# JvanZyl1/PSSO-SAC-for-powered-descent

Measured on AMD Instinct MI355X. Metric: env-steps/sec at 65 536 parallel envs; achieved HBM GB/s vs peak, higher is better.
Workload: dtype f64; 1 GPU; c3: 65536 envs/GPU, landing_burn_pure_throttle, rtd_rl reward, wind (percentile profile drawn per reset + VK gusts below 15 km) + tilt, auto-reset, uniform random actions; synchronized starts, 640 untimed burn-in + 5 warmup steps; envs_per_gpu=65536, global_envs=65536, parallelism=env-shard x1

## Files before the change

### include/pdenv.h

```cpp
#ifndef PDENV_H
#define PDENV_H
#include <stddef.h>
#include <stdint.h>

#ifdef __cplusplus
extern "C" {
#endif

#define PD_ABI_VERSION 11
#define PD_MAX_PTS 256
#define PD_MAX_COLS 5
#define PD_MAX_TAB 64
#define PD_MAX_WIND 16
#define PD_N_WIND_PROFILES 50
#define PD_N_STATE 11
#define PD_N_INFO 49
#define PD_ACTOR_PARAMS_PURE_THROTTLE 249
#define PD_ACTOR_PARAMS_LANDING_BURN 372

typedef enum { PD_OK = 0, PD_ERR_INVALID = 1, PD_ERR_HIP = 2, PD_ERR_NOMEM = 3, PD_ERR_UNSUPPORTED = 4 } pd_status;
typedef enum {
    PD_PHASE_PURE_THROTTLE = 0, PD_PHASE_LANDING_BURN = 1, PD_PHASE_PCONTROL = 2,
    PD_PHASE_BALLISTIC_ARC = 3, PD_PHASE_FLIP_OVER = 4, PD_PHASE_SUBSONIC = 5, PD_PHASE_SUPERSONIC = 6,
    PD_PHASE_LANDING_BURN_ACS = 7
} pd_phase;
typedef enum { PD_RTD_RL = 0, PD_RTD_PSO = 1, PD_RTD_NONE = 2 } pd_rtd;
typedef enum { PD_F64 = 0, PD_F32 = 1 } pd_precision;
typedef enum { PD_INTEG_REFERENCE = 0, PD_INTEG_RK4 = 1 } pd_integrator;
typedef enum {
    PD_TABLES_NO_CELL_PIECES = 1,
    PD_TABLES_NO_FINE_INDEX = 2,
    PD_TABLES_EXACT_ATMOSPHERE = 4,
    PD_TABLES_VERBOSE = 8,
    PD_TABLES_NO_CARRY = 16,
    PD_TABLES_NO_ATM_LDS = 32
} pd_table_flags;

typedef struct {
    int32_t n_cols, n_pts;
    double col_aoa[PD_MAX_COLS];
    int32_t col_start[PD_MAX_COLS], col_len[PD_MAX_COLS];
    double mach[PD_MAX_PTS];
    double coef[PD_MAX_PTS];
} pd_aero_table;

typedef struct {
    double thrust_per_engine, nozzle_exit_pressure, nozzle_exit_area, v_exhaust;
    int32_t n_engines_gimballed, pad0;
    double grid_fin_area, d_base_grid_fin, rocket_radius, frontal_area, m_prop0, C_gust_x, C_gust_y;
    double h_ox, h_f, m_ox, m_f, h_lower, m_dry, x_dry, I_dry, engine_height, cop;
    double isa_Hb[9], isa_Tb[9], isa_beta[9], isa_pb[9];
    double isa_g0, isa_R, isa_kappa, isa_r, isa_alt_max, grav_R, grav_g0;
    pd_aero_table cd, cl;
    int32_t ca_n, cn_n;
    double ca_x[PD_MAX_TAB], ca_y[PD_MAX_TAB], ca_min_mach, ca_min_val;
    double cn_x[PD_MAX_TAB], cn_y[PD_MAX_TAB], cn_min_mach, cn_max_mach, cn_min_val, cn_max_val, cn_slope;
    int32_t wind_n[PD_N_WIND_PROFILES];
    double wind_alt_km[PD_N_WIND_PROFILES][PD_MAX_WIND], wind_speed[PD_N_WIND_PROFILES][PD_MAX_WIND];
    double vk_Ad_u[4], vk_Bd_u[2], vk_Ad_v[4], vk_Bd_v[2], vk_y_threshold;
    double sigma_u_lo, sigma_u_hi, sigma_v_lo, sigma_v_hi;
    double state0[PD_N_STATE];
    double norm_y, norm_vy, norm_x, norm_vx;
    const uint64_t* keys_cd; int64_t n_keys_cd;
    const uint64_t* keys_cl; int64_t n_keys_cl;
    double full_rocket[13];
    double cop_ascent;
    int32_t n_engines_stage1, pad1;
    double rcs_force, rcs_d_bottom, rcs_d_top;
// ... 183 lines not shown
```

### psso-sac-for-powered-descent_amd/csrc/kstep.hip

```cpp
#include "pd_step_impl.h"

#if !defined(PD_KR) || !defined(PD_KPH) || !defined(PD_KW)
#error "kstep.hip needs -DPD_KR=0|1 -DPD_KPH=0|1|2 -DPD_KW=0|1"
#endif

namespace pd {
#if PD_KR == 0
using KR = double;
#else
using KR = float;
#endif
constexpr bool KW = PD_KW != 0;

#define PD_INST_STEP(RT)                                                          \
    template void launch_step<KR, PD_KPH, RT, KW, 1>(const StepArgs<KR>&, hipStream_t);  \
    template void launch_step<KR, PD_KPH, RT, KW, 2>(const StepArgs<KR>&, hipStream_t);  \
    template void launch_step<KR, PD_KPH, RT, KW, 4>(const StepArgs<KR>&, hipStream_t);  \
    template void launch_step<KR, PD_KPH, RT, KW, 8>(const StepArgs<KR>&, hipStream_t);  \
    template void launch_step<KR, PD_KPH, RT, KW, 16>(const StepArgs<KR>&, hipStream_t);

#if defined(PD_KROLL)
static_assert(PD_KPH < 2, "SAC rollout unit: the two landing burns");
#if PD_KROLL == 2
template void launch_sac_collect<KR, PD_KPH, KW>(const StepArgs<KR>&, hipStream_t);
#else
template void launch_sac_roll<KR, PD_KPH, KW>(const StepArgs<KR>&, hipStream_t);
#endif
#elif defined(PD_KRK4)
static_assert(PD_KPH == 0 && PD_KW == 0, "RK4 unit: pure throttle without wind");
template void launch_step<KR, 0, 0, false, 2, true>(const StepArgs<KR>&, hipStream_t);
template void launch_step<KR, 0, 0, false, 16, true>(const StepArgs<KR>&, hipStream_t);
template void launch_step<KR, 0, 1, false, 2, true>(const StepArgs<KR>&, hipStream_t);
template void launch_step<KR, 0, 1, false, 16, true>(const StepArgs<KR>&, hipStream_t);
#elif defined(PD_KLPE)
template void launch_step<KR, PD_KPH, 0, KW, PD_KLPE>(const StepArgs<KR>&, hipStream_t);
#else
PD_INST_STEP(0)
#endif
#if PD_KPH < 2 && !defined(PD_KLPE) && !defined(PD_KRK4) && !defined(PD_KROLL)
PD_INST_STEP(1)
template void launch_policy_lpe<KR, PD_KPH, KW, 2>(const StepArgs<KR>&, int64_t, hipStream_t);
template void launch_policy_lpe<KR, PD_KPH, KW, 4>(const StepArgs<KR>&, int64_t, hipStream_t);
template void launch_policy_lpe<KR, PD_KPH, KW, 8>(const StepArgs<KR>&, int64_t, hipStream_t);
#endif
}
```

### psso-sac-for-powered-descent_amd/csrc/pd_step.h

```cpp
#pragma once
#include <hip/hip_runtime.h>

#include <cstring>

#include "../../include/pdenv.h"
#include "pd_physics.h"
#include "pd_sac_mlp.h"

namespace pd {

constexpr int kBlock = 256;
constexpr int kStepBlock = 256;
#ifndef PD_WG512
#define PD_WG512 1
#endif
#ifndef PD_ATM_LDS
#define PD_ATM_LDS 1
#endif
#ifndef PD_WIND_SLOPE
#define PD_WIND_SLOPE 1
#endif
#ifndef PD_MERGE
#define PD_MERGE 2
#endif
template <typename R, int PHASE, bool WIND, int LPE, int POL, bool RK4, bool SAC> constexpr bool step_big() {
    return PD_WG512 != 0 && sizeof(R) == 8 && PHASE == 0 && WIND && LPE == 2 && POL == 0 && !RK4 && !SAC;
}
template <typename R, int PHASE, bool WIND, int LPE, int POL, bool RK4, bool SAC> constexpr int step_block() {
    return step_big<R, PHASE, WIND, LPE, POL, RK4, SAC>() ? 512 : kStepBlock;
}
constexpr int kScratch = kSys * kSys + kSys + 3 * kNbr + kPay;
constexpr int kPendingCap = 4096;
constexpr int kSolveSlots = 1024;
constexpr int kGridExact = 1 << 30;
constexpr int kGridRefine = 1 << 29;
constexpr int kGridBisect = 1 << 28;
constexpr int kGridPiece = 1 << 27;
constexpr uint32_t kFinePiece = 1u << 30;
constexpr uint32_t kFineBisect = 1u << 29;
constexpr uint32_t kFineRefined = 1u << 28;
constexpr uint32_t kFineIndex = kFineRefined - 1u;

constexpr int kCellDeg = 8;
constexpr int kCellCoef = (kCellDeg + 1) * (kCellDeg + 2) / 2;
constexpr int kCellExact = 4;
constexpr int kCellKey = kCellCoef + 3 * kCellExact;
constexpr int kCellStride = (kCellKey + 2) & ~1;
constexpr int kCellKeyF = (kCellKey + 1) & ~1;
constexpr int kCellStrideF = (kCellKeyF + 2 + 3) & ~3;
template <typename R> constexpr int cell_stride() { return sizeof(R) == 8 ? kCellStride : kCellStrideF; }
template <typename R> constexpr int cell_key() { return sizeof(R) == 8 ? kCellKey : kCellKeyF; }

struct GridBisect {
    double nx, ny, c, tau;
    unsigned long long key_a, key_b;
    int slot_a, slot_b;
// ... 136 lines not shown
    unsigned int* ticket;
};

template <typename R>
__device__ void insert_pending(unsigned long long* count, const unsigned long long* pkeys, const double* ppay,
                               unsigned long long* stats, unsigned long long* keys_cd, R* pay_cd, int lc_cd,
                               unsigned long long* keys_cl, R* pay_cl, int lc_cl) {
    unsigned long long cnt = *count;
    if (cnt == 0) return;
    if (cnt > (unsigned long long)kPendingCap) cnt = kPendingCap;
    for (unsigned long long e = 0; e < cnt; ++e) {
        const unsigned long long kk = pkeys[e];
        const int table = (int)(kk >> 63);
        const unsigned long long key = kk & ~(1ull << 63);
        unsigned long long* keys = table ? keys_cl : keys_cd;
        const int lc = table ? lc_cl : lc_cd;
        uint32_t mask = (1u << lc) - 1u, h = key_hash(key, lc);
        int slot = -1;
        for (uint32_t p = 0; p <= mask; ++p) {
            const unsigned long long k = keys[h];
            if (k == key) { slot = -1; break; }
            if (k == kEmptyKey) { slot = (int)h; break; }
            h = (h + 1) & mask;
        }
        if (slot >= 0 && stats[kStInsCd + table] * 2 + 2 > (1ull << lc)) slot = -1;
        if (slot < 0) continue;
        stats[kStInsCd + table] += 1;
        keys[slot] = key;
        pay_store<R>(ppay + e * kPay, (table ? pay_cl : pay_cd) + (int64_t)slot * pay_stride<R>());
    }
    *count = 0;
}

constexpr int kArgCount = 1, kArgNoCarry = 2;
constexpr int kRollOff = 0, kRollEpisodes = 1, kRollCollect = 2;
template <typename R> struct StepArgs {
    uint64_t P;
    EnvBufs<R> b;
    Pending pend;
    int64_t n;
    uint64_t env_offset;
    uint32_t seed_lo, seed_hi;
    int act_f64, auto_reset, stochastic, fixed_prof, use_tilt;
    double tilt_sigma;
    const void* actions;
    R* obs; R* reward; uint8_t* done; uint8_t* trunc; int8_t* trunc_id;
    const double* noise;
    R* info;
    uint64_t info_mask;
    int info_nsel;
    R* reward_sum;
    const float* policy_w;
    const int32_t* list_in; int32_t* list_out;
    const uint32_t* cnt_in; uint32_t* cnt_out; uint32_t* cnt_zero;
    int use_list;
    double dt_aux;
    int rtd_none;
    int n_fused;
    int count_work;
    const float* sac_mean; const float* sac_logstd; const float* sac_eps;
    float sac_lo, sac_hi, sac_max;
    uint32_t sac_hs;
    float* sac_act; float* slab; float* obs32;
    int sac_draw;
    float* sac_eps_out;
    int64_t ring_cap;
    long long* ring_state;
// ... 21 lines not shown
```

### psso-sac-for-powered-descent_amd/csrc/pd_step_impl.h

```cpp
#pragma once
#include "pd_envdev.h"

namespace pd {

__device__ __forceinline__ int dpp_swap1(int v) { return __builtin_amdgcn_mov_dpp(v, 0xB1, 0xF, 0xF, false); }
__device__ __forceinline__ float pair_swap(float v) { return __int_as_float(dpp_swap1(__float_as_int(v))); }
__device__ __forceinline__ double pair_swap(double v) {
    const uint64_t b = (uint64_t)__double_as_longlong(v);
    const uint32_t lo = (uint32_t)dpp_swap1((int)(uint32_t)b), hi = (uint32_t)dpp_swap1((int)(uint32_t)(b >> 32));
    return __longlong_as_double((long long)(((uint64_t)hi << 32) | lo));
}

template <int LPE, typename R>
__device__ __forceinline__ void sincos_pair(R x0, R x1, int role, R& s0, R& c0, R& s1, R& c1) {
    if constexpr (LPE >= 2) {
        const bool odd = role & 1;
        R s, c;
        pd_sincos<R>(odd ? x1 : x0, s, c);
        const R so = pair_swap(s), co = pair_swap(c);
        s0 = odd ? so : s; c0 = odd ? co : c;
        s1 = odd ? s : so; c1 = odd ? c : co;
    } else {
        pd_sincos<R>(x0, s0, c0);
        pd_sincos<R>(x1, s1, c1);
    }
}
template <int LPE, typename R>
__device__ __forceinline__ void div_pair(R a0, R b0, R a1, R b1, int role, R& q0, R& q1) {
    if constexpr (LPE >= 2) {
        const bool odd = role & 1;
        const R q = (odd ? a1 : a0) / (odd ? b1 : b0);
        const R qo = pair_swap(q);
        q0 = odd ? qo : q; q1 = odd ? q : qo;
    } else {
        q0 = a0 / b0; q1 = a1 / b1;
    }
// ... 592 lines not shown
        run(g, b0);
        if (k + 1 < K) {
            fetch(gidx(k + 2), b0);
            run(g + NQ, b1);
        }
    }
    if (halfr) {
        const bool odd = K & 1;
        R hp[10];
        uint32_t hwd[3];
#pragma unroll
        for (int u = 0; u < 10; ++u) hp[u] = odd ? b1.pp[u] : b0.pp[u];
#pragma unroll
        for (int u = 0; u < 3; ++u) hwd[u] = odd ? b1.w[u] : b0.w[u];
        const R hsum = chunk_half<R, R2>(hp, hwd, odd ? b1.pt : b0.pt, odd ? b1.M : b0.M, odd ? b1.a : b0.a, lane & 1);
        wave_lds_sync();
        B.qm[lane] = hsum;
        wave_lds_sync();
        if (lane < rem) B.part[Kfull * NQ + lane] = B.qm[2 * lane] + B.qm[2 * lane + 1];
    }
    wave_lds_sync();
    R val = R(0);
    if (mine) {
        const R* pr = B.part + kChunks * rank;
        R tot = pr[0];
#pragma unroll
        for (int c = 1; c < kChunks; ++c) tot = tot + pr[c];
        val = rbf_finish_f<R>(pf, tot, M, aq);
    }
    wave_lds_sync();
    return val;
}

template <typename R, typename Pre, typename AT>
__device__ __forceinline__ R rbf2(const AT& a, DP<R>& P, int table, const TabView<R>& t, const LineLds<R>& ln,
                                  RbfCache<R>& cache, R M, R aq, bool act, BalLds<R>& B, const R* tab,
                                  WaveCount& wc, Pre&& pre, unsigned long long* stamp = nullptr) {
#ifdef PD_STAMP
    const unsigned long long s0 = __builtin_amdgcn_s_memtime();
#endif
    TayRef tr{-1, 0, false, false, false, false, -1, 0.0, 0.0, false};
    const int slot = rbf_lookup<R>(a, P, table, t, ln, cache, M, aq, &tr, stamp ? stamp + 2 : nullptr, pre);
#ifdef PD_STAMP
    const unsigned long long s1 = __builtin_amdgcn_s_memtime();
    stamp[0] += s1 - s0;
#endif
    const bool tay = act && tr.piece >= 0;
    const bool cel = act && tr.cp >= 0;
    const bool full = act && !tay && !cel && slot >= 0;
    R vt = R(0);
    R vb;
    if (sizeof(R) == 8 || t.cell_pc != nullptr) {
        if (tay) vt = taylor_eval<R>(gbl(P.tay) + (size_t)tr.piece * kTayStride, M, tr.cell);
        if (cel) {
            const PD_AS1 R* rec = t.cell_pc + (size_t)tr.cp * cell_stride<R>();
            vt = cell_eval<R>(rec, M, aq, (R)tr.cu, (R)tr.cv);
            if (tr.fine) cache.key = *(const PD_AS1 unsigned long long*)(rec + cell_key<R>());
        }
        vb = rbf_balanced<R>(P, B, tab, full, table, slot, M, aq, []() {});
    } else {
        vb = rbf_balanced<R>(P, B, tab, full, table, slot, M, aq, [&]() {
            if (tay) vt = taylor_eval<R>(gbl(P.tay) + (size_t)tr.piece * kTayStride, M, tr.cell);
        });
    }
    R val = full ? vb : vt;
#ifdef PD_STAMP
    const unsigned long long s2 = __builtin_amdgcn_s_memtime();
    stamp[1] += s2 - s1;
#endif
    const bool miss = act && !tay && !cel && slot < 0;
    if (wc.w) {
        const int nf = __popcll(__ballot(full));
        wc.add(kStQLine - kStWork, act && tr.line);
        wc.add(kStQVerify - kStWork, act && tr.verify);
        wc.add(kStQTaylor - kStWork, tay);
        wc.add(kStQCell - kStWork, cel);
        wc.add_n(kStQBal - kStWork, nf);
        wc.add(kStQMiss - kStWork, miss);
        wc.add_n(kStBalRounds - kStWork, (kChunks * nf + 63) >> 6);
        wc.add(kStQRefined - kStWork, act && tr.refined);
        wc.add(kStQBisect - kStWork, act && tr.bisect);
        wc.add_n(kStWRefined - kStWork, __ballot(act && tr.refined) != 0ull);
        wc.add_n(kStWBisect - kStWork, __ballot(act && tr.bisect) != 0ull);
        wc.add_n(kStWMixed - kStWork, (__ballot(act && tr.line) != 0ull) && (__ballot(act && !tr.line) != 0ull));
    }
    if (__ballot(miss)) {
        R mv = rbf_miss_wave<R>(a, P, table, t.smach, cache.key, M, aq, 0, 1, miss);
        if (miss) val = mv;
    }
    return val;
}

template <typename R> __device__ __forceinline__ R cd_query(R ae) {
    R aoa = ae * Cst<R>::rad2deg;
    const R r10 = (R)(10.0 * kDeg2Rad);
    if (aoa > r10) aoa = r10;
    else if (aoa < (R)(-10.0 * kDeg2Rad)) aoa = (R)(-10.0 * kDeg2Rad);
    return aoa;
}
template <typename R> __device__ __forceinline__ R cl_query(R ae, R& sgn, bool& zero) {
    R aq = (ae * Cst<R>::rad2deg) * Cst<R>::rad2deg;
    sgn = R(1);
    zero = false;
    if (aq > R(10)) aq = R(10);
    else if (aq < R(-10)) aq = R(-10);
    else if (fabs(aq) < R(1e-6)) zero = true;
    else if (aq < R(0)) { aq = fabs(aq); sgn = R(-1); }
    return aq;
}

template <int IN, int NL, int OUT, bool SPLIT = false>
__device__ __forceinline__ void actor_forward(const float* __restrict__ W, int64_t N, uint32_t ui,
                                              int half, const float* x, float* y) {
    constexpr int H = 8;
    constexpr int HS = SPLIT ? H / 2 : H;
    constexpr bool OSPLIT = SPLIT && OUT % 2 == 0;
    constexpr int OS = OSPLIT ? OUT / 2 : OUT;
    static_assert((HS * IN) % 4 == 0 && (H * IN) % 4 == 0, "layer-1 blocks of whole chunks");
    using F4 = __attribute__((ext_vector_type(4))) float;
// ... 130 lines not shown
    t.keys = gbl(table ? P.keys_cl : P.keys_cd);
    t.pay = gbl(table ? P.pay_cl : P.pay_cd);
    t.logcap = table ? P.logcap_cl : P.logcap_cd;
    t.line0 = table ? 2 : 0;
    t.grid_key = gbl(P.grid_key[table]);
    t.grid_slot = gbl(P.grid_slot[table]);
    t.sub_key = gbl(P.sub_key[table]);
    t.sub_slot = gbl(P.sub_slot[table]);
    t.sub_bis = gbl((const GridBisect*)P.sub_bis[table]);
    t.cell_pc = gbl(P.cell_pc[table]);
    t.sub_piece = gbl(P.sub_piece[table]);
    t.fine = gbl(P.fine[table]);
    t.grid_nm = P.grid_nm[table];
    t.grid_na = P.grid_na[table];
    t.grid_a0 = P.grid_a0[table];
    t.grid_inv_da = P.grid_inv_da[table];
    t.grid_inv_dm = P.grid_inv_dm[table];
    return t;
}

template <typename R, int PHASE, int RTD, bool WIND, int LPE, int POL = 0, bool RK4 = false, bool CNT = false,
          bool SAC = false, int ROLL = kRollOff>
__global__ __launch_bounds__((step_block<R, PHASE, WIND, LPE, POL, RK4, SAC>()))
__attribute__((amdgpu_waves_per_eu(2))) void k_step(StepArgs<R> a_) {
    SA<R>& a = kargs<R>();
    static_assert(sizeof(a_) > 0);
    static_assert(!ROLL || (SAC && LPE == 16 && !POL && !RK4 && !CNT && RTD == 0 && PHASE <= 1),
                  "ROLL: the SAC kernel of the RL landing burns at 16 lanes per env");
    constexpr int kStepBlock = step_block<R, PHASE, WIND, LPE, POL, RK4, SAC>();
    constexpr bool kBig = step_big<R, PHASE, WIND, LPE, POL, RK4, SAC>();
    constexpr int EPB = kStepBlock / LPE;
    constexpr bool kEpi = ROLL == kRollEpisodes, kCol = ROLL == kRollCollect;
    __shared__ StepLds<R, WIND, EPB, LPE == 2, CNT, kStepBlock, kBig> L;
#ifdef PD_STAMP
    unsigned long long acc_[17] = {};
#endif
    PD_T(t_start);
    int64_t n_act = a.n;
    constexpr bool kRefill = POL && !WIND;
    int64_t ring_pos0 = 0;
    if constexpr (SAC) { if (a.ring_state) ring_pos0 = (int64_t)__atomic_load_n(a.ring_state, __ATOMIC_RELAXED); }
    if constexpr (POL) {
        if (blockIdx.x == 0 && threadIdx.x == 0) *a.cnt_zero = 0u;
        if (kRefill && a.refill) n_act = a.refill_slots;
        if (a.use_list) {
            n_act = (int64_t)*a.cnt_in;
            if ((int64_t)blockIdx.x * EPB >= n_act) return;
        }
    }
    const int64_t N = a.n;
    const int64_t gt = (int64_t)blockIdx.x * kStepBlock + threadIdx.x;
    bool valid = gt / LPE < n_act;
    const bool slot = valid;
    bool drained = false;
    int64_t e_act = valid ? gt / LPE : n_act - 1;
    int rq_next = 0;
    if constexpr (kRefill) {
        if (a.refill && valid) {
            constexpr int kEpw = 64 / LPE;
            const int64_t gw = gt >> 6;
            e_act = gw * (int64_t)a.refill_q + (int64_t)(((int)gt & 63) / LPE);
            rq_next = kEpw;
        }
    }
    int64_t i = (POL && a.use_list) ? (int64_t)a.list_in[e_act] : e_act;
    const int role = (int)(gt % LPE);
// ... 63 lines not shown
            else if (t < kImg + kLog) stg[k] = lgt[t - kImg];
        }
    }
    constexpr bool kSacMlp = SAC && LPE == 16;
    __shared__ __attribute__((aligned(16))) float s_mlp[kSacMlp ? sac_mlp_lds_floats<256>() : 1];
    __shared__ float s_sach[kSacMlp ? kSacTile * 16 : 1];
    __shared__ float s_obs[ROLL ? kSacTile * 16 : 1];
    if constexpr (kSacMlp && !ROLL) {
        const int H = a.sac_mlp.H;
        if (H) {
            const int64_t e0 = (int64_t)blockIdx.x * kSacTile;
            const int A2 = a.sac_mlp.A;
            auto put = [&](int e, int o, float v) {
                s_sach[e * 16 + (o < A2 ? o : 8 + o - A2)] = v;
                if (a.sac_heads_out && e0 + e < a.n) a.sac_heads_out[(e0 + e) * 2 * A2 + o] = v;
            };
            if (H == 128) sac_mlp_tile<128>(a.sac_mlp, a.n, e0, s_mlp, put);
            else sac_mlp_tile<256>(a.sac_mlp, a.n, e0, s_mlp, put);
            __syncthreads();
        }
    }
    {
        DP<R>& P = *params<R>(a.P);
#pragma unroll
        for (int k = 0; k < kPer; ++k) {
            const int t = threadIdx.x + k * kStepBlock;
            if (t < kImg) ((V4*)static_cast<StepStatic<R, WIND, kBig>*>(&L))[t] = stg[k];
            else if (t < kImg + kLog) ((V4*)s_logtab)[t - kImg] = stg[k];
        }
        if constexpr (CNT) { if (threadIdx.x < (kStepBlock / 64) * kNWork) (&L.work[0][0])[threadIdx.x] = 0u; }
        if (threadIdx.x < 2) L.tdesc[threadIdx.x] = tab_view<R>(P, L.tab, (int)threadIdx.x);
    }
    __syncthreads();
    PD_T(t_staged);
    PD_ACC(0, t_staged - t_start);
    if constexpr (POL) {
        if (!a.use_list && __ballot(live) == 0) return;
    }
    const int aux = PHASE == 2 ? params<R>(a.P)->phase : PHASE;
    const bool ascent = PHASE == 2 && (aux == PD_PHASE_SUBSONIC || aux == PD_PHASE_SUPERSONIC);
    constexpr int A = PHASE == 0 ? 1 : (PHASE == 1 ? 4 : 2);
    const int AD = PHASE == 2 ? (ascent ? 2 : 1) : A;
    static_assert(!RK4 || (PHASE == 0 && !WIND && !POL), "RK4: pure throttle, no wind, no policy");
    constexpr int NSUB = RK4 ? 40 : (PHASE == 2 ? 1 : 4);
#ifndef PD_CARRY_WIDE
#define PD_CARRY_WIDE 0
#endif
    constexpr bool kSpills = RK4 && LPE == 16;
    constexpr bool kCarry = (PD_CARRY & 3) != 0 && (PD_CARRY_WIDE || (sizeof(R) == 8 && !kSpills && !SAC));
    constexpr bool kActAhead = (PD_CARRY & 4) != 0 && !POL && !SAC &&
                               (PD_CARRY_WIDE || (PHASE == 0 && sizeof(R) == 8 && !kSpills));
    constexpr bool kMergeDiv = (PD_MERGE & 2) != 0 && !CNT && LPE == 2 && sizeof(R) == 8 && PHASE <= 1 && !RK4 && !SAC &&
                               !POL;
    constexpr bool kAtmTab = sizeof(R) == 4 || !WIND;
    constexpr bool kAtmLds = kBig && PD_ATM_LDS != 0;
    constexpr bool kWindSlope = kBig && PD_WIND_SLOPE != 0;
    constexpr bool kPcs = !WIND && !RK4 && LPE <= 8 && (PHASE == 0 || (PHASE == 1 && !SAC));
    const R dt = RK4 ? R(0.01) : (PHASE == 0 ? R(0.025) : (PHASE == 1 ? R(0.1) : (R)a.dt_aux));
    const R dt_act = PHASE == 2 ? dt : R(0.025);
    PD_T(t_loaded);
    PD_ACC(1, t_loaded - t_staged);

    auto store_all = [&]() {
    uint32_t uo = ui;
    asm volatile("" : "+v"(uo));
    if (live) {
// ... 52 lines not shown
    WaveCount wc{CNT ? L.work[threadIdx.x >> 6] : nullptr};
    R k_rho = R(0), k_patm = R(0), k_asnd = R(0);
    double k_speed = 0.0;
    bool k_have = false;
    using RS = double;
    RS xs[sizeof(R) == 8 ? 1 : 11];
    auto SV = [&](int k) -> RS& {
        if constexpr (sizeof(R) == 8) return e.s[k];
        else return xs[k];
    };
    uint32_t an0[kActAhead ? A : 1], an1[kActAhead ? A : 1];
    auto act_request = [&](int fr) {
        if constexpr (kActAhead) {
            SA<R>& a = kargs<R>();
            const size_t fo = (size_t)fr * (size_t)N;
            if (a.act_f64) {
#pragma unroll
                for (int k = 0; k < A; ++k) if (k < AD) {
                    const unsigned long long w = (unsigned long long)__double_as_longlong(
                        ldv((const double*)a.actions + fo * AD + k, ui * AD));
                    an0[k] = (uint32_t)w; an1[k] = (uint32_t)(w >> 32);
                }
            } else {
#pragma unroll
                for (int k = 0; k < A; ++k) if (k < AD) an0[k] = __float_as_uint(ldv((const float*)a.actions + fo * AD + k, ui * AD));
            }
        }
    };
    if constexpr (kActAhead) {
#pragma unroll
        for (int k = 0; k < A; ++k) { an0[k] = 0u; an1[k] = 0u; }
        if (nf > 0) act_request(0);
    }
#pragma unroll 1
    for (int f = 0; f < nf; ++f) {
    SA<R>& a = kargs<R>();
    const size_t fo = (size_t)f * (size_t)N;
    float uf[A];
    double ud[A];
#pragma unroll
    for (int k = 0; k < A; ++k) { uf[k] = 0.f; ud[k] = 0.0; }
    if constexpr (ROLL) {
        if (role == 0) {
            DP<R>& Q = *params<R>(a.P);
            constexpr int ok = PHASE == 0 ? 0 : 3;
            obs_eval<R>(Q, ok, e.s, [&](int k, R v) { s_obs[le * obs_dim(ok) + k] = (float)v; });
        }
        if (!__syncthreads_or(live ? 1 : 0)) break;
        const int A2 = a.sac_mlp.A;
        auto put = [&](int en, int o, float v) { s_sach[en * 16 + (o < A2 ? o : 8 + o - A2)] = v; };
        if (a.sac_mlp.H == 128) sac_mlp_tile<128>(a.sac_mlp, a.n, (int64_t)blockIdx.x * kSacTile, s_mlp, put, NoMark{}, s_obs);
        else sac_mlp_tile<256>(a.sac_mlp, a.n, (int64_t)blockIdx.x * kSacTile, s_mlp, put, NoMark{}, s_obs);
        __syncthreads();
    }
    if (!ROLL || __ballot(live) != 0ull) {
    if constexpr (POL) {
        DP<R>& Q = *params<R>(a.P);
        uint32_t uw = wcopy ? (uint32_t)e_act : ui;
        asm volatile("" : "+v"(uw));
        const float* W = wcopy ? a.policy_wc : a.policy_w;
        if constexpr (PHASE == 0) {
            float x[2] = {(float)(e.s[1] / Q.norm_y), (float)(e.s[3] / Q.norm_vy)};
            actor_forward<2, 3, 1, (LPE >= 2)>(W, N, uw, role & 1, x, uf);
        } else {
            float x[5] = {(float)(e.s[0] / Q.norm_x), (float)(e.s[1] / Q.norm_y), (float)(e.s[2] / Q.norm_vx),
                          (float)(e.s[3] / Q.norm_vy), (float)tanh(Q.k_theta_pso * (e.s[4] - Cst<R>::pi / R(2)))};
            actor_forward<5, 4, 4, (LPE >= 2)>(W, N, uw, role & 1, x, uf);
        }
    } else if constexpr (SAC) {
// ... 59 lines not shown
        const uint32_t W = 2u * (uint32_t)obs_dim(ok) + (uint32_t)AD + 2u;
        obs_eval<R>(Q, ok, e.s, [&](int k, R v) { ev(a.slab, srow * W + (uint32_t)k) = (float)v; });
        if (a.prio) ev(a.prio, srow) = *a.max_prio;
    }
    R gdeg_out = e.act0, dcmdl_out = e.act1, dcmdr_out = e.act2;
    const R gprev = e.act0, dlprev = e.act1, drprev = e.act2;
    bool nan_hit = false;
    const bool tap = a.info != nullptr && role == 0 && live;
    auto info = [&](int k, R v) {
        const uint64_t m = a.info_mask;
        if (!((m >> k) & 1ull)) return;
        const size_t row = (size_t)f * (size_t)a.info_nsel + (size_t)__popcll(m & ((1ull << k) - 1ull));
        uint32_t u = ui;
        uint32_t blo = (uint32_t)(uint64_t)a.info, bhi = (uint32_t)((uint64_t)a.info >> 32);
        asm volatile("" : "+v"(u), "+s"(blo), "+s"(bhi));
        R* base = (R*)(((uint64_t)bhi << 32) | blo);
        ev(base + row * (size_t)N, u) = v;
    };

    bool wpre = false;
    RS rkb[8], rka[8];
    if constexpr (sizeof(R) == 4) {
#pragma unroll
        for (int k = 0; k < 11; ++k) xs[k] = (RS)e.s[k];
    }
    const RS dts = RK4 ? 0.01 : (PHASE == 0 ? 0.025 : (PHASE == 1 ? 0.1 : a.dt_aux));
#pragma unroll 1
    for (int sub = 0; sub < NSUB; ++sub) {
        PD_T(t_sub);
        const int stage = RK4 ? (sub & 3) : 0;
        SA<R>& a = kargs<R>();
        DP<R>& P = *params<R>(a.P);
        const bool tap_sub = tap && sub == NSUB - 1;
        if constexpr (kCarry) { if (a.count_work & kArgNoCarry) carry = kCarryNone; }
        RS x = SV(0), y = SV(1), vx = SV(2), vy = SV(3), th = SV(4), thd = SV(5), ga = SV(6), al = SV(7);
        RS m = SV(8), mp = SV(9);
        if constexpr (WIND) wc.add(kStGust - kStWork, role == 0 && live && a.stochastic && y < P.vk_y_threshold);
        R rho, patm, asnd;
        RS speed;
        if (RK4 ? (sub == 0 && k_have) : k_have) { rho = k_rho; patm = k_patm; asnd = k_asnd; speed = k_speed; }
        else {
            if constexpr (kAtmLds) atmosphere_lds<R>(P, L.isa, L.atl, (R)y, rho, patm, asnd);
            else atmosphere<R, kAtmTab>(P, L.isa, (R)y, rho, patm, asnd);
            speed = sqrt(vx * vx + vy * vy);
        }
        const R spR = (R)speed;
        R mach = R(0);
        R x_prop = R(0);
        if constexpr (kMergeDiv) {
            R fpc0 = div_known<R>((R)(P.m_prop0 - mp), P.m_prop0, P.inv_m_prop0, P.div2 & kDiv2MProp0);
            if (fpc0 == R(0)) fpc0 = R(1e-6);
            R xp_num, xp_den, mr;
            inertia_x_prop<R>(P, R(1) - fpc0, xp_num, xp_den);
            div_pair<LPE, R>(spR, asnd, xp_num, xp_den, role, mr, x_prop);
            if (asnd != R(0)) mach = (R(10) < mr) ? R(10) : mr;
        } else {
            if (asnd != R(0)) { R mr = spR / asnd; mach = (R(10) < mr) ? R(10) : mr; }
        }
        const R ae = (R)((vy < RS(0)) ? ga - th - Cst<RS>::pi : al);
        R ug = R(0), vg = R(0);
        auto wind_block = [&]() {
            if constexpr (WIND) {
                const R* walt = L.walt + e.prof * 16;
                const R* wsp = L.wsp + e.prof * 16;
                R km = PD_DIVC(R, (R)y, 1000);
                int wn = P.wind_n[e.prof];
// ... 33 lines not shown
                    if (!drawn) {
                        u32x4 r = philox_k({(uint32_t)g, (uint32_t)(g >> 32) ^ e.ep, e.ts, kTagWindSub + (uint32_t)sub},
                                         a.seed_lo, a.seed_hi);
                        gauss_pair(r, lic, llc, w0, w1);
                    }
                    R n0 = (P.vk_Ad_u[0] * e.fu0 + P.vk_Ad_u[1] * e.fu1) + (e.sgu * P.vk_Bd_u[0]) * (R)w0;
                    R n1 = (P.vk_Ad_u[2] * e.fu0 + P.vk_Ad_u[3] * e.fu1) + (e.sgu * P.vk_Bd_u[1]) * (R)w0;
                    e.fu0 = n0; e.fu1 = n1;
                    n0 = (P.vk_Ad_v[0] * e.fv0 + P.vk_Ad_v[1] * e.fv1) + (e.sgv * P.vk_Bd_v[0]) * (R)w1;
                    n1 = (P.vk_Ad_v[2] * e.fv0 + P.vk_Ad_v[3] * e.fv1) + (e.sgv * P.vk_Bd_v[1]) * (R)w1;
                    e.fv0 = n0; e.fv1 = n1;
                    ug = ug + e.fu1;
                    vg = e.fv1;
                }
                wpre = gust && (sub & 1) == 0;
            }
        };
        R CL = R(0), CD = R(0);
        PD_T(t_aero0);
        PD_ACC(2, t_aero0 - t_sub);
        {
            R cl_sgn; bool cl_zero;
            R aq_cl = cl_query<R>(ae, cl_sgn, cl_zero);
            R aq_cd = cd_query<R>(ae);
            const bool have = asnd != R(0);
            if constexpr (LPE == 1) {
                R v = rbf<kPcs, R>(a, P, 1, tab_view_lds<R>(L.tdesc, 1), L.lines, cB, mach, aq_cl, 0, 1);
                R w = rbf<kPcs, R>(a, P, 0, tab_view_lds<R>(L.tdesc, 0), L.lines, cA, mach, aq_cd, 0, 1);
                CL = (!have || cl_zero) ? R(0) : (cl_sgn < R(0) ? -v : v);
                CD = have ? w : R(0);
            } else {
                R v;
                if constexpr (LPE == 2)
                    v = rbf2<R>(a, P, my_table, tab_view_lds<R>(L.tdesc, my_table), L.lines, cA, mach,
                                my_table ? aq_cl : aq_cd, live, L.bal[threadIdx.x >> 6], L.tab, wc, wind_block
#ifdef PD_STAMP
                                , acc_ + 7
#endif
                                );
                else
                    v = rbf<kPcs, R>(a, P, my_table, tab_view_lds<R>(L.tdesc, my_table), L.lines, cA, mach,
                                     my_table ? aq_cl : aq_cd, part, nparts);
                if constexpr (nparts >= 2) v += __shfl_xor(v, 1);
                if constexpr (nparts >= 4) v += __shfl_xor(v, 2);
                if constexpr (nparts >= 8) v += __shfl_xor(v, 4);
                R vcd, vcl;
                if constexpr (LPE == 2) {
                    const R vo = pair_swap(v);
                    vcd = role ? vo : v; vcl = role ? v : vo;
                } else {
                    vcd = __shfl(v, gbase);
                    vcl = __shfl(v, gbase + nparts);
                }
                CD = have ? vcd : R(0);
                CL = (!have || cl_zero) ? R(0) : (cl_sgn < R(0) ? -vcl : vcl);
            }
        }
        PD_T(t_aero1);
        PD_ACC(3, t_aero1 - t_aero0);
        R q = R(0.5) * rho * (spR * spR);
        RS mp_l = mp;
        if constexpr (kMergeDiv) asm volatile("" : "+v"(mp_l));
        R fpc = div_known<R>((R)(P.m_prop0 - mp_l), P.m_prop0, P.inv_m_prop0, P.div2 & kDiv2MProp0);
        if (fpc == R(0)) fpc = R(1e-6);
        R x_cog, I;
        R grq_m = R(0);
        if constexpr (kMergeDiv) {
// ... 530 lines not shown
                if (slot && !live && rank < take) {
                    const int64_t nx = (gt >> 6) * (int64_t)a.refill_q + (int64_t)(rq_next + rank);
                    e_act = nx; i = nx; ui = (uint32_t)nx; g = a.env_offset + (uint64_t)nx; valid = true;
                    load_env();
                    live = true;
                    k_have = false;
                }
                rq_next += take;
            }
        }
        if (kRefill && a.refill && !drained && rq_next >= a.refill_q) {
            const unsigned long long mk = __ballot(slot && !live && role == 0);
            const int nw = __popcll(mk);
            if (nw >= a.refill || (nw > 0 && __ballot(live) == 0ull)) {
                const int lane = (int)__lane_id();
                const int leader = __ffsll((long long)mk) - 1;
                uint32_t base = 0;
                if (lane == leader) base = atomicAdd(a.refill_next, (uint32_t)nw);
                base = (uint32_t)__shfl((int)base, leader);
                drained = (int64_t)a.refill_base + (int64_t)base + nw >= N;
                const int64_t nx = (int64_t)a.refill_base + (int64_t)base + (int64_t)__popcll(mk & ((1ull << gbase) - 1ull));
                if (slot && !live && nx < N) {
                    e_act = nx; i = nx; ui = (uint32_t)nx; g = a.env_offset + (uint64_t)nx; valid = true;
                    load_env();
                    live = true;
                    k_have = false;
                }
            }
        }
        if (__ballot(live) == 0ull) break;
    }
    }
    }
    if constexpr (POL) {
        const bool cont = role == 0 && live;
        const unsigned long long mk = __ballot(cont);
        if (mk) {
            const int lane = (int)__lane_id();
            const int leader = __ffsll((long long)mk) - 1;
            uint32_t base = 0;
            if (lane == leader) base = atomicAdd(a.cnt_out, (uint32_t)__popcll(mk));
            base = (uint32_t)__shfl((int)base, leader);
            if (cont) a.list_out[base + (uint32_t)__popcll(mk & ((1ull << lane) - 1ull))] = (int32_t)i;
        }
    }

    PD_T(t_store);
    if constexpr (kEpi) { if (live) roll_store(a.roll_t0 + nf, 0, e.tid, false); }
    store_all();
    if constexpr (SAC) {
        if (a.ring_state) {
            __syncthreads();
            if (threadIdx.x == 0) {
                const unsigned long long t = atomicAdd((unsigned long long*)&a.ring_state[2], 1ull);
                if (t == (unsigned long long)gridDim.x - 1ull) {
                    const int64_t adv = kCol ? (int64_t)nf * N : N;
                    const int64_t np = ring_pos0 + adv, sz = (int64_t)a.ring_state[1] + adv;
                    a.ring_state[0] = (long long)(np >= a.ring_cap ? np - a.ring_cap : np);
                    a.ring_state[1] = (long long)(sz > a.ring_cap ? a.ring_cap : sz);
                    a.ring_state[2] = 0;
                }
            }
        }
    }
    if constexpr (!POL) {
        __syncthreads();
        if (threadIdx.x == 0) {
            const unsigned int t = atomicAdd(a.pend.ticket, 1u);
            if (t == gridDim.x - 1u) {
                __threadfence();
                DP<R>& P = *params<R>(a.P);
                insert_pending<R>(a.pend.count, a.pend.keys, a.pend.pay, a.pend.stats, (unsigned long long*)P.keys_cd, (R*)P.pay_cd, P.logcap_cd,
                                  (unsigned long long*)P.keys_cl, (R*)P.pay_cl, P.logcap_cl);
                *a.pend.ticket = 0u;
            }
        }
    }
    if (wc.w && __lane_id() == 0) {
#pragma unroll
        for (int k = 0; k < kNWork; ++k)
            if (wc.w[k]) atomicAdd(&a.pend.stats[kStWork + k], (unsigned long long)wc.w[k]);
    }
// ... 54 lines not shown
```

### psso-sac-for-powered-descent_amd/csrc/pdenv.hip

```cpp
#include <hip/hip_runtime.h>

#include <algorithm>
#include <array>
#include <cstdio>
#include <cstdlib>
#include <cstring>
#include <map>
#include <memory>
#include <mutex>
#include <string>
#include <vector>

#include "../../include/pdenv.h"
#include "pd_envdev.h"
#include "pd_tables.h"

using namespace pd;

namespace pd {
thread_local std::string g_err;
pd_status set_error(pd_status s, const char* m) { g_err = m; return s; }
}

namespace {
// ... 154 lines not shown
int act_dim_of(int phase) {
    return phase == PD_PHASE_LANDING_BURN ? 4 : ((phase == PD_PHASE_SUBSONIC || phase == PD_PHASE_SUPERSONIC) ? 2 : 1);
}
}

namespace {

pd_status dalloc(pd_env* e, void** p, size_t bytes) {
    if (bytes == 0) bytes = 8;
    PD_HIP(hipMalloc(p, bytes));
    e->allocs.push_back(*p);
    return PD_OK;
}

template <typename R> StepArgs<R> make_args(pd_env* e) {
    StepArgs<R> a{};
    a.P = (uint64_t)e->dparams;
    a.b.st = (R*)e->st; a.b.vprev = (R*)e->vprev; a.b.gwin = (R*)e->gwin; a.b.ghead = e->ghead; a.b.glen = e->glen;
    a.b.act = (R*)e->act; a.b.wind = (R*)e->wind; a.b.wprof = e->wprof; a.b.key = e->key; a.b.slot = e->slot;
    a.b.tid = e->tid; a.b.epi = e->epi; a.b.tstep = e->tstep; a.b.fin = e->fin;
    a.pend = e->pend;
    a.n = e->cfg.n_envs;
    a.env_offset = e->cfg.env_offset;
    a.seed_lo = (uint32_t)e->cfg.seed; a.seed_hi = (uint32_t)(e->cfg.seed >> 32);
    a.act_f64 = e->cfg.action_f64;
    a.auto_reset = e->cfg.auto_reset;
    a.stochastic = e->cfg.stochastic_wind;
    a.fixed_prof = e->cfg.wind_percentile >= 50 ? e->cfg.wind_percentile - 50 : -1;
    a.use_tilt = e->cfg.tilt_sigma_rad > 0.0;
    a.tilt_sigma = e->cfg.tilt_sigma_rad;
    a.dt_aux = e->cfg.dt > 0.0 ? e->cfg.dt : 0.1;
    a.rtd_none = e->cfg.rtd == PD_RTD_NONE;
    a.n_fused = 1;
    a.count_work = (e->count_work ? kArgCount : 0) | ((e->cfg.table_flags & PD_TABLES_NO_CARRY) ? kArgNoCarry : 0);
    return a;
}

template <typename F> auto with_real(bool f64, F&& f) {
    if (f64) return f(double{});
    return f(float{});
}
template <typename F> auto with_real(const pd_env* e, F&& f) { return with_real(e->rsize == 8, f); }

pd_status validate(const pd_params* p, const pd_config* c) {
    if (!p || !c) return fail(PD_ERR_INVALID, "null params/config");
    if (c->n_envs <= 0 || c->n_envs > (int64_t)1 << 25) return fail(PD_ERR_INVALID, "n_envs out of range (1 .. 2^25 per handle)");
    if (c->phase < 0 || c->phase > PD_PHASE_LANDING_BURN_ACS) return fail(PD_ERR_INVALID, "bad phase");
    if (c->rtd != PD_RTD_RL && c->rtd != PD_RTD_PSO && c->rtd != PD_RTD_NONE) return fail(PD_ERR_INVALID, "bad rtd");
    if (c->phase == PD_PHASE_LANDING_BURN_ACS)
        return fail(PD_ERR_UNSUPPORTED, "landing_burn_ACS: the reference raises TypeError at its first step "
                                        "(rockets_physics.py:867-891 passes ACS arguments to the gimballed decomposer; "
                                        "base_environment.py:126-130 passes two prevs to a three-prev lambda)");
    if (c->rtd == PD_RTD_RL && c->phase == PD_PHASE_FLIP_OVER)
        return fail(PD_ERR_UNSUPPORTED, "flip_over_boostbackburn with rtd RL: the reference raises TypeError at its first "
                                        "step (rtd_rl.py:134 truncated_func(state) called with three arguments, "
                                        "base_environment.py:150); use PD_RTD_NONE for physics stepping");
    if (c->rtd == PD_RTD_PSO && c->phase > PD_PHASE_LANDING_BURN)
        return fail(PD_ERR_UNSUPPORTED, "rtd PSO exists for the two landing burns only: the other rtd_pso functions take "
                                        "(state) / (state, done, truncated) and raise TypeError when the env calls them "
                                        "(rtd_pso.py:38,63,107,120,141,157 vs base_environment.py:150-152)");
    if (c->dt < 0.0) return fail(PD_ERR_INVALID, "dt must be >= 0");
    if (c->rtd == PD_RTD_RL && (c->phase == PD_PHASE_LANDING_BURN || c->phase == PD_PHASE_PCONTROL) &&
        (c->trajectory_length < 1 || !(c->discount_factor > 0.0 && c->discount_factor < 1.0)))
        return fail(PD_ERR_INVALID, "this RL reward needs discount_factor in (0, 1) and trajectory_length >= 1");
    if (c->phase == PD_PHASE_SUBSONIC || c->phase == PD_PHASE_SUPERSONIC) {
        if (!p->ref_y || !p->ref_x || !p->ref_vx || !p->ref_vy || p->n_ref < 2)
            return fail(PD_ERR_INVALID, "ascent phases need the reference trajectory (ref_y/x/vx/vy, n_ref >= 2)");
    }
    if (c->precision != PD_F64 && c->precision != PD_F32) return fail(PD_ERR_INVALID, "bad precision");
    if (c->integrator != PD_INTEG_REFERENCE && c->integrator != PD_INTEG_RK4) return fail(PD_ERR_INVALID, "bad integrator");
    if (c->table_flags & ~(PD_TABLES_NO_CELL_PIECES | PD_TABLES_NO_FINE_INDEX | PD_TABLES_EXACT_ATMOSPHERE | PD_TABLES_VERBOSE |
                           PD_TABLES_NO_CARRY | PD_TABLES_NO_ATM_LDS))
        return fail(PD_ERR_INVALID, "unknown table_flags bits");
    if (c->integrator == PD_INTEG_RK4 && (c->phase != PD_PHASE_PURE_THROTTLE || c->enable_wind))
        return fail(PD_ERR_UNSUPPORTED, "the RK4 integrator (non-parity, BASELINE c2) exists for "
                                        "landing_burn_pure_throttle without wind only");
    for (const pd_aero_table* t : {&p->cd, &p->cl})
        for (int k = 0; k < t->n_cols; ++k)
            if (!(t->col_aoa[k] >= 0.0 && t->col_aoa[k] <= 255.0 && t->col_aoa[k] == (double)(int)t->col_aoa[k]))
                return fail(PD_ERR_INVALID, "aero table column AoAs must be integers in [0, 255]");
    if (c->action_f64 && c->precision != PD_F64) return fail(PD_ERR_INVALID, "f64 actions need PD_F64");
    if (c->enable_wind && !(c->wind_percentile == -1 || (c->wind_percentile >= 50 && c->wind_percentile <= 99)))
        return fail(PD_ERR_INVALID, "wind_percentile must be 50..99 or -1");
    const pd_aero_table* ts[2] = {&p->cd, &p->cl};
    for (auto t : ts) {
        if (t->n_cols != kCols || t->n_pts < kNbr || t->n_pts > PD_MAX_PTS) return fail(PD_ERR_INVALID, "aero table shape");
        int s = 0;
        for (int k = 0; k < kCols; ++k) {
            if (t->col_start[k] != s || t->col_len[k] < 1 || t->col_len[k] >= (1 << kKeyLoBits))
                return fail(PD_ERR_INVALID, "aero column layout");
            s += t->col_len[k];
        }
        if (s != t->n_pts) return fail(PD_ERR_INVALID, "aero column count");
    }
    if (p->ca_n < 2 || p->ca_n > PD_MAX_TAB || p->cn_n < 2 || p->cn_n > PD_MAX_TAB) return fail(PD_ERR_INVALID, "grid fin tables");
    for (int w = 0; w < PD_N_WIND_PROFILES; ++w)
        if (c->enable_wind && (p->wind_n[w] < 1 || p->wind_n[w] > PD_MAX_WIND)) return fail(PD_ERR_INVALID, "wind profile");
    return PD_OK;
}

template <typename T, typename P> pd_status upload(pd_env* e, const T* src, size_t n, P** dev) {
    void* d;
    pd_status st = dalloc(e, &d, n * sizeof(T));
    if (st != PD_OK) return st;
    if (n) PD_HIP(hipMemcpy(d, src, n * sizeof(T), hipMemcpyHostToDevice));
// ... 1118 lines not shown
```

### psso-sac-for-powered-descent_amd/pdenv/_lib.py

```python
import ctypes as C
import os

HERE = os.path.dirname(os.path.abspath(__file__))
LIB_PATH = os.path.join(HERE, "libpdenv.so")

D, I32, I64, U64 = C.c_double, C.c_int32, C.c_int64, C.c_uint64
MAX_PTS, MAX_COLS, MAX_TAB, MAX_WIND, N_PROF = 256, 5, 64, 16, 50
N_STATE, N_INFO = 11, 49

PD_OK, PD_ERR_INVALID, PD_ERR_HIP, PD_ERR_NOMEM, PD_ERR_UNSUPPORTED = range(5)
(PURE_THROTTLE, LANDING_BURN, PCONTROL, BALLISTIC_ARC, FLIP_OVER, SUBSONIC, SUPERSONIC,
 LANDING_BURN_ACS) = range(8)
RTD_RL, RTD_PSO, RTD_NONE = 0, 1, 2
F64, F32 = 0, 1
ACTOR_PARAMS = {0: 249, 1: 372}

INFO_FIELDS = ["air_density", "atmospheric_pressure", "speed_of_sound", "mach_number",
               "dynamic_pressure", "CL", "CD", "mass_flow", "x_cog", "inertia",
               "alpha_effective", "throttle", "g_load_1_sec_window", "ug", "vg", "gimbal_angle_deg",
               "mach_number_max", "drag", "lift", "d_cp_cg", "d_thrust_cg", "fuel_percentage_consumed",
               "control_force_parallel", "control_force_perpendicular", "control_force_x", "control_force_y",
               "aero_force_x", "aero_force_y", "gravity", "F_wind_x", "F_wind_y", "vx_dot", "vy_dot",
               "control_moment_z", "aero_moment_z", "M_wind_z", "moments_z", "theta_dot_dot",
               "delta_command_left_rad", "delta_command_right_rad", "delta_left_rad", "delta_right_rad",
# ... 20 lines not shown
        ("grav_R", D), ("grav_g0", D),
        ("cd", PdAeroTable), ("cl", PdAeroTable),
        ("ca_n", I32), ("cn_n", I32),
        ("ca_x", D * MAX_TAB), ("ca_y", D * MAX_TAB), ("ca_min_mach", D), ("ca_min_val", D),
        ("cn_x", D * MAX_TAB), ("cn_y", D * MAX_TAB), ("cn_min_mach", D), ("cn_max_mach", D),
        ("cn_min_val", D), ("cn_max_val", D), ("cn_slope", D),
        ("wind_n", I32 * N_PROF),
        ("wind_alt_km", (D * MAX_WIND) * N_PROF), ("wind_speed", (D * MAX_WIND) * N_PROF),
        ("vk_Ad_u", D * 4), ("vk_Bd_u", D * 2), ("vk_Ad_v", D * 4), ("vk_Bd_v", D * 2), ("vk_y_threshold", D),
        ("sigma_u_lo", D), ("sigma_u_hi", D), ("sigma_v_lo", D), ("sigma_v_hi", D),
        ("state0", D * N_STATE), ("norm_y", D), ("norm_vy", D), ("norm_x", D), ("norm_vx", D),
        ("keys_cd", C.POINTER(U64)), ("n_keys_cd", I64),
        ("keys_cl", C.POINTER(U64)), ("n_keys_cl", I64),
        ("full_rocket", D * 13), ("cop_ascent", D), ("n_engines_stage1", I32), ("pad1", I32),
        ("rcs_force", D), ("rcs_d_bottom", D), ("rcs_d_top", D),
        ("state0_phase", (D * N_STATE) * 8), ("norm_phase", (D * 8) * 8),
        ("ref_y", C.POINTER(D)), ("ref_x", C.POINTER(D)), ("ref_vx", C.POINTER(D)), ("ref_vy", C.POINTER(D)),
        ("n_ref", I32), ("pad2", I32),
        ("hyper", ((D * 9) * 12) * 2), ("terminal_mach", D * 2),
    ]


class PdConfig(C.Structure):
    _fields_ = [("n_envs", I64), ("device", I32), ("phase", I32), ("rtd", I32), ("precision", I32),
                ("seed", U64), ("env_offset", U64), ("enable_wind", I32), ("stochastic_wind", I32),
                ("wind_percentile", I32), ("auto_reset", I32), ("tilt_sigma_rad", D),
                ("action_f64", I32), ("lanes_per_env", I32),
                ("dt", D), ("discount_factor", D), ("trajectory_length", I32), ("integrator", I32),
                ("table_flags", I32), ("pad3", I32)]


TABLES_NO_CELL_PIECES, TABLES_NO_FINE_INDEX, TABLES_EXACT_ATMOSPHERE, TABLES_VERBOSE, TABLES_NO_CARRY = 1, 2, 4, 8, 16
TABLES_NO_ATM_LDS = 32


class PdTuning(C.Structure):
    _fields_ = [("step_fuse", I32), ("policy_fuse", I32), ("policy_lanes", I32), ("policy_list", I32),
                ("policy_list_at", D), ("policy_refill", I32), ("policy_slots", I32),
                ("policy_refill_own", I32), ("pad_tuning", I32)]


EXPORTS = ["pd_abi_version", "pd_sizeof_params", "pd_sizeof_config", "pd_last_error", "pd_device_count", "pd_create",
           "pd_destroy", "pd_reset", "pd_step", "pd_step_n", "pd_rollout", "pd_rollout_policy", "pd_pso_step",
           "pd_flush_misses", "pd_observe", "pd_get_state", "pd_set_state", "pd_get_actuators", "pd_set_actuators",
           "pd_set_gload_window", "pd_get_gload_window", "pd_set_wind_sigmas", "pd_get_wind_state",
           "pd_set_wind_state", "pd_get_counters", "pd_set_counters", "pd_checkpoint_size", "pd_checkpoint_save",
           "pd_checkpoint_load", "pd_counters", "pd_stats", "pd_count_work", "pd_atmosphere", "pd_obs_dim",
           "pd_action_dim", "pd_step_sac", "pd_pso_swarm_minima", "pd_pso_update_bests", "pd_cell_piece_info",
           "pd_step_sac_ring", "pd_sac_actor", "pd_step_sac_fused", "pd_atm_table", "pd_set_tuning", "pd_get_tuning",
           "pd_pso_swarm_minima_scratch_bytes", "pd_step_n_info", "pd_pso_step_chunked", "pd_rollout_policy_chunked",
           "pd_rollout_sac", "pd_atm_table_lds", "pd_wind_slopes", "pd_collect_sac", "pd_per_sample_scratch_bytes",
           "pd_per_sample", "pd_per_update", "pd_sac_critic", "pd_sac_td_target"]
PER_MAX_BATCH = 1024
ABI_VERSION = 11

_lib = None


class PdError(RuntimeError):
    pass


def load(path=None):
    global _lib
    if _lib is not None:
        return _lib
# ... 103 lines not shown
```

Baseline: 2.354 billion env-steps/s.

## Pace paired waves on the same SIMD via dynamic s_setprio

```diff
diff --git a/include/pdenv.h b/include/pdenv.h
--- a/include/pdenv.h
+++ b/include/pdenv.h
@@ -33,7 +33,8 @@
     PD_TABLES_EXACT_ATMOSPHERE = 4,
     PD_TABLES_VERBOSE = 8,
     PD_TABLES_NO_CARRY = 16,
-    PD_TABLES_NO_ATM_LDS = 32
+    PD_TABLES_NO_ATM_LDS = 32,
+    PD_TABLES_NO_PACE = 64
 } pd_table_flags;
 
 typedef struct {
diff --git a/psso-sac-for-powered-descent_amd/csrc/kstep.hip b/psso-sac-for-powered-descent_amd/csrc/kstep.hip
--- a/psso-sac-for-powered-descent_amd/csrc/kstep.hip
+++ b/psso-sac-for-powered-descent_amd/csrc/kstep.hip
@@ -44,3 +44,11 @@
 template void launch_policy_lpe<KR, PD_KPH, KW, 8>(const StepArgs<KR>&, int64_t, hipStream_t);
 #endif
 }
+
+#if defined(PD_WAVE_TIMES) && PD_KR == 0 && PD_KPH == 0 && PD_KW == 1 && !defined(PD_KROLL) && !defined(PD_KRK4) && \
+    !defined(PD_KLPE)
+extern "C" int pd_debug_wave_times(void* out, int n) {
+    if (n < 0 || n > pd::kWaveRecWaves) return (int)hipErrorInvalidValue;
+    return (int)hipMemcpyFromSymbol(out, HIP_SYMBOL(pd::g_wave_rec), (size_t)n * pd::kWaveRec * 8, 0, hipMemcpyDeviceToHost);
+}
+#endif
diff --git a/psso-sac-for-powered-descent_amd/csrc/pd_step.h b/psso-sac-for-powered-descent_amd/csrc/pd_step.h
--- a/psso-sac-for-powered-descent_amd/csrc/pd_step.h
+++ b/psso-sac-for-powered-descent_amd/csrc/pd_step.h
@@ -22,6 +22,9 @@
 #endif
 #ifndef PD_MERGE
 #define PD_MERGE 2
+#endif
+#ifndef PD_PACE
+#define PD_PACE 1
 #endif
 template <typename R, int PHASE, bool WIND, int LPE, int POL, bool RK4, bool SAC> constexpr bool step_big() {
     return PD_WG512 != 0 && sizeof(R) == 8 && PHASE == 0 && WIND && LPE == 2 && POL == 0 && !RK4 && !SAC;
@@ -224,7 +227,7 @@
     *count = 0;
 }
 
-constexpr int kArgCount = 1, kArgNoCarry = 2;
+constexpr int kArgCount = 1, kArgNoCarry = 2, kArgNoPace = 4;
 constexpr int kRollOff = 0, kRollEpisodes = 1, kRollCollect = 2;
 template <typename R> struct StepArgs {
     uint64_t P;
diff --git a/psso-sac-for-powered-descent_amd/csrc/pd_step_impl.h b/psso-sac-for-powered-descent_amd/csrc/pd_step_impl.h
--- a/psso-sac-for-powered-descent_amd/csrc/pd_step_impl.h
+++ b/psso-sac-for-powered-descent_amd/csrc/pd_step_impl.h
@@ -2,6 +2,11 @@
 #include "pd_envdev.h"
 
 namespace pd {
+
+#ifdef PD_WAVE_TIMES
+constexpr int kWaveRec = 16, kWaveRecWaves = 16384;
+static __device__ unsigned long long g_wave_rec[kWaveRecWaves * kWaveRec];
+#endif
 
 __device__ __forceinline__ int dpp_swap1(int v) { return __builtin_amdgcn_mov_dpp(v, 0xB1, 0xF, 0xF, false); }
 __device__ __forceinline__ float pair_swap(float v) { return __int_as_float(dpp_swap1(__float_as_int(v))); }
@@ -660,7 +665,7 @@
     return val;
 }
 
-template <typename R, typename Pre, typename AT>
+template <typename R, bool PACE = false, typename Pre, typename AT>
 __device__ __forceinline__ R rbf2(const AT& a, DP<R>& P, int table, const TabView<R>& t, const LineLds<R>& ln,
                                   RbfCache<R>& cache, R M, R aq, bool act, BalLds<R>& B, const R* tab,
                                   WaveCount& wc, Pre&& pre, unsigned long long* stamp = nullptr) {
@@ -713,6 +718,7 @@
         wc.add_n(kStWMixed - kStWork, (__ballot(act && tr.line) != 0ull) && (__ballot(act && !tr.line) != 0ull));
     }
     if (__ballot(miss)) {
+        if constexpr (PACE) __builtin_amdgcn_s_setprio(0);
         R mv = rbf_miss_wave<R>(a, P, table, t.smach, cache.key, M, aq, 0, 1, miss);
         if (miss) val = mv;
     }
@@ -909,6 +915,21 @@
     constexpr int EPB = kStepBlock / LPE;
     constexpr bool kEpi = ROLL == kRollEpisodes, kCol = ROLL == kRollCollect;
     __shared__ StepLds<R, WIND, EPB, LPE == 2, CNT, kStepBlock, kBig> L;
+    constexpr int kPaceBits = kBig ? (PD_PACE) : 0;
+    constexpr bool kPaceSub = (kPaceBits & 2) != 0, kPaceFb = (kPaceBits & 3) != 0;
+    constexpr bool kPaceFlip = !kPaceFb && (kPaceBits & 4) != 0;
+    constexpr unsigned kPaceFin = 0xffffffffu;
+    __shared__ unsigned s_pace[kPaceFb ? 32 : 1];
+    using PaceWord = volatile __attribute__((address_space(3))) unsigned;
+    if constexpr (kPaceFb) {
+        unsigned hw;
+        asm volatile("s_getreg_b32 %0, hwreg(HW_REG_HW_ID)" : "=s"(hw));
+        ((PaceWord*)s_pace)[threadIdx.x >> 6] = (hw >> 4) & 3u;
+        ((PaceWord*)s_pace)[8 + (threadIdx.x >> 6)] = 0u;
+    }
+#ifdef PD_WAVE_TIMES
+    const unsigned long long wt0_ = __builtin_amdgcn_s_memrealtime();
+#endif
 #ifdef PD_STAMP
     unsigned long long acc_[17] = {};
 #endif
@@ -1038,6 +1059,26 @@
         if (threadIdx.x < 2) L.tdesc[threadIdx.x] = tab_view<R>(P, L.tab, (int)threadIdx.x);
     }
     __syncthreads();
+    if constexpr (kPaceFb) {
+        const int wv = (int)(threadIdx.x >> 6);
+        constexpr int kWv = kStepBlock / 64;
+        PaceWord* sp = (PaceWord*)s_pace;
+        const unsigned mine = sp[wv];
+        int cnt = 0, peer = -1;
+#pragma unroll
+        for (int k = 0; k < kWv; ++k) {
+            const bool same = k != wv && sp[k] == mine;
+            cnt += same ? 1 : 0;
+            peer = same ? k : peer;
+        }
+        const bool paced = cnt == 1 && !(a.count_work & kArgNoPace);
+        sp[16 + wv] = 8u + (unsigned)(paced ? peer : wv);
+#ifdef PD_WAVE_TIMES
+        sp[24 + wv] = (unsigned)(paced ? peer : -1);
+#endif
+    }
+    bool pace_flip = false;
+    if constexpr (kPaceFlip) pace_flip = !(a.count_work & kArgNoPace);
     PD_T(t_staged);
     PD_ACC(0, t_staged - t_start);
     if constexpr (POL) {
@@ -1156,9 +1197,39 @@
         for (int k = 0; k < A; ++k) { an0[k] = 0u; an1[k] = 0u; }
         if (nf > 0) act_request(0);
     }
+    auto pace = [&](unsigned begun) {
+        if constexpr (kPaceFb) {
+            PaceWord* sp = (PaceWord*)s_pace;
+            const unsigned wv = threadIdx.x >> 6;
+            const unsigned peer = sp[16 + wv] & 15u;
+            sp[8 + wv] = begun;
+            const unsigned pf = (unsigned)__builtin_amdgcn_readfirstlane((int)sp[peer]);
+            if (pf != kPaceFin && pf > begun) __builtin_amdgcn_s_setprio(1);
+            else __builtin_amdgcn_s_setprio(0);
+        }
+    };
+#ifdef PD_WAVE_TIMES
+    const unsigned wt_wid_ = blockIdx.x * (kStepBlock / 64) + (threadIdx.x >> 6);
+    auto wt_sample = [&](int done) {
+        if constexpr (kBig) {
+            if (done && !(done & 15) && done <= 128 && __lane_id() == 0 && wt_wid_ < (unsigned)kWaveRecWaves)
+                g_wave_rec[(size_t)wt_wid_ * kWaveRec + 4 + (done >> 4)] = __builtin_amdgcn_s_memrealtime();
+        }
+    };
+#endif
 #pragma unroll 1
     for (int f = 0; f < nf; ++f) {
     SA<R>& a = kargs<R>();
+#ifdef PD_WAVE_TIMES
+    wt_sample(f);
+#endif
+    if constexpr (kPaceFb && !kPaceSub) pace((unsigned)f + 1u);
+    if constexpr (kPaceFlip) {
+        if (pace_flip) {
+            if (__builtin_amdgcn_readfirstlane((f ^ (int)(threadIdx.x >> 8)) & 1)) __builtin_amdgcn_s_setprio(1);
+            else __builtin_amdgcn_s_setprio(0);
+        }
+    }
     const size_t fo = (size_t)f * (size_t)N;
     float uf[A];
     double ud[A];
@@ -1284,6 +1355,7 @@
         SA<R>& a = kargs<R>();
         DP<R>& P = *params<R>(a.P);
         const bool tap_sub = tap && sub == NSUB - 1;
+        if constexpr (kPaceSub) pace((unsigned)(NSUB * f + sub) + 1u);
         if constexpr (kCarry) { if (a.count_work & kArgNoCarry) carry = kCarryNone; }
         RS x = SV(0), y = SV(1), vx = SV(2), vy = SV(3), th = SV(4), thd = SV(5), ga = SV(6), al = SV(7);
         RS m = SV(8), mp = SV(9);
@@ -1383,7 +1455,7 @@
             } else {
                 R v;
                 if constexpr (LPE == 2)
-                    v = rbf2<R>(a, P, my_table, tab_view_lds<R>(L.tdesc, my_table), L.lines, cA, mach,
+                    v = rbf2<R, (kPaceFb || kPaceFlip)>(a, P, my_table, tab_view_lds<R>(L.tdesc, my_table), L.lines, cA, mach,
                                 my_table ? aq_cl : aq_cd, live, L.bal[threadIdx.x >> 6], L.tab, wc, wind_block
 #ifdef PD_STAMP
                                 , acc_ + 7
@@ -1980,6 +2052,13 @@
     }
     }
     }
+    if constexpr (kPaceFb || kPaceFlip) {
+        if constexpr (kPaceFb) ((PaceWord*)s_pace)[8 + (threadIdx.x >> 6)] = kPaceFin;
+        __builtin_amdgcn_s_setprio(0);
+    }
+#ifdef PD_WAVE_TIMES
+    wt_sample(nf);
+#endif
     if constexpr (POL) {
         const bool cont = role == 0 && live;
         const unsigned long long mk = __ballot(cont);
@@ -1996,6 +2075,22 @@
     PD_T(t_store);
     if constexpr (kEpi) { if (live) roll_store(a.roll_t0 + nf, 0, e.tid, false); }
     store_all();
+#ifdef PD_WAVE_TIMES
+    if constexpr (kBig) {
+        __builtin_amdgcn_s_waitcnt(0);
+        const unsigned long long wt1_ = __builtin_amdgcn_s_memrealtime();
+        unsigned hw, xcc;
+        asm volatile("s_getreg_b32 %0, hwreg(HW_REG_HW_ID)" : "=s"(hw));
+        asm volatile("s_getreg_b32 %0, hwreg(HW_REG_XCC_ID)" : "=s"(xcc));
+        if (__lane_id() == 0 && wt_wid_ < (unsigned)kWaveRecWaves) {
+            unsigned long long* rec = g_wave_rec + (size_t)wt_wid_ * kWaveRec;
+            rec[0] = wt0_; rec[1] = wt1_; rec[2] = hw; rec[3] = xcc; rec[4] = threadIdx.x >> 6;
+            long long peer = -1;
+            if constexpr (kPaceFb) peer = (long long)(int)((PaceWord*)s_pace)[24 + (threadIdx.x >> 6)];
+            rec[13] = (unsigned long long)peer;
+        }
+    }
+#endif
     if constexpr (SAC) {
         if (a.ring_state) {
             __syncthreads();
diff --git a/psso-sac-for-powered-descent_amd/csrc/pdenv.hip b/psso-sac-for-powered-descent_amd/csrc/pdenv.hip
--- a/psso-sac-for-powered-descent_amd/csrc/pdenv.hip
+++ b/psso-sac-for-powered-descent_amd/csrc/pdenv.hip
@@ -210,7 +210,8 @@
     a.dt_aux = e->cfg.dt > 0.0 ? e->cfg.dt : 0.1;
     a.rtd_none = e->cfg.rtd == PD_RTD_NONE;
     a.n_fused = 1;
-    a.count_work = (e->count_work ? kArgCount : 0) | ((e->cfg.table_flags & PD_TABLES_NO_CARRY) ? kArgNoCarry : 0);
+    a.count_work = (e->count_work ? kArgCount : 0) | ((e->cfg.table_flags & PD_TABLES_NO_CARRY) ? kArgNoCarry : 0) |
+                   ((e->cfg.table_flags & PD_TABLES_NO_PACE) ? kArgNoPace : 0);
     return a;
 }
 
@@ -248,7 +249,7 @@
     if (c->precision != PD_F64 && c->precision != PD_F32) return fail(PD_ERR_INVALID, "bad precision");
     if (c->integrator != PD_INTEG_REFERENCE && c->integrator != PD_INTEG_RK4) return fail(PD_ERR_INVALID, "bad integrator");
     if (c->table_flags & ~(PD_TABLES_NO_CELL_PIECES | PD_TABLES_NO_FINE_INDEX | PD_TABLES_EXACT_ATMOSPHERE | PD_TABLES_VERBOSE |
-                           PD_TABLES_NO_CARRY | PD_TABLES_NO_ATM_LDS))
+                           PD_TABLES_NO_CARRY | PD_TABLES_NO_ATM_LDS | PD_TABLES_NO_PACE))
         return fail(PD_ERR_INVALID, "unknown table_flags bits");
     if (c->integrator == PD_INTEG_RK4 && (c->phase != PD_PHASE_PURE_THROTTLE || c->enable_wind))
         return fail(PD_ERR_UNSUPPORTED, "the RK4 integrator (non-parity, BASELINE c2) exists for "
diff --git a/psso-sac-for-powered-descent_amd/pdenv/_lib.py b/psso-sac-for-powered-descent_amd/pdenv/_lib.py
--- a/psso-sac-for-powered-descent_amd/pdenv/_lib.py
+++ b/psso-sac-for-powered-descent_amd/pdenv/_lib.py
@@ -76,6 +76,7 @@
 
 TABLES_NO_CELL_PIECES, TABLES_NO_FINE_INDEX, TABLES_EXACT_ATMOSPHERE, TABLES_VERBOSE, TABLES_NO_CARRY = 1, 2, 4, 8, 16
 TABLES_NO_ATM_LDS = 32
+TABLES_NO_PACE = 64
 
 
 class PdTuning(C.Structure):
```

Measured after the change: 2.479 billion env-steps/s, median of 6. 5.3% higher.
